# p2004dr/visual-slam

Hardware: AMD Instinct MI355X
Metric: frames/sec (extract+match+pose) at 640×480, 2000 ORB, 1/2/4/8 MI355X (higher is better)
Workload: dtype u8

## Files before the change

### visual-slam_amd/csrc/ctx.hip

```cpp
#include <algorithm>
#include <cmath>
#include <cstring>
#include <vector>

#include <cstdlib>

#include "common.h"

int mo_fail(mo_ctx* c, int code, const std::string& msg) {
    if (c) c->err = msg;
    return code;
}

static std::string g_create_err;

extern "C" int mo_abi_version(void) { return MO_ABI_VERSION; }

extern "C" int mo_device_count(void) {
    int n = 0;
    if (hipGetDeviceCount(&n) != hipSuccess) return 0;
    return n;
}

extern "C" mo_ctx* mo_create(int device, int max_w, int max_h, int max_batch) {
// ... 104 lines not shown
        float v = 0;
        hipEventElapsedTime(&v, t.ev[i], t.ev[i + 1]);
        ms[i] = v;
    }
    t.names[t.n_stages] = nullptr;
    if (names) *names = t.names;
    return n;
}

extern "C" int mo_stage_times(mo_ctx* c, const char*** names, float* ms, int cap) { return mo_stage_times_back(c, 0, names, ms, cap); }

static bool params_equal(const mo_orb_params& a, const mo_orb_params& b) {
    return std::memcmp(&a, &b, sizeof(a)) == 0;
}

static int fill_plan(mo_ctx* c, const mo_orb_params* p, int w, int h, int batch);

int mo_build_plan(mo_ctx* c, const mo_orb_params* p, int w, int h, int batch) {
    if (!p) return mo_fail(c, MO_ERR_ARG, "params is NULL");
    if (w < 64 || h < 64 || w > c->max_w || h > c->max_h)
        return mo_fail(c, MO_ERR_ARG, "image size outside the context's max_w/max_h (or < 64)");
    if (batch < 1 || batch > c->max_batch) return mo_fail(c, MO_ERR_ARG, "batch outside 1..max_batch");
    if (p->nlevels < 1 || p->nlevels > MO_MAX_LEVELS) return mo_fail(c, MO_ERR_ARG, "nlevels must be 1..12");
    if (p->first_level != 0 || p->wta_k != 2 || p->score_type != 0 || p->patch_size != 31)
        return mo_fail(c, MO_ERR_UNSUPPORTED,
                       "only firstLevel=0, WTA_K=2, HARRIS_SCORE, patchSize=31 (the reference's values) are built");
    if (p->edge_threshold < 19 || p->edge_threshold > 1024)
        return mo_fail(c, MO_ERR_UNSUPPORTED, "edge_threshold must be >= 19 (descriptor radius)");
    if (p->nfeatures < 1 || !(p->scale_factor > 1.0f) || p->scale_factor > 2.0f)
        return mo_fail(c, MO_ERR_ARG, "nfeatures >= 1, 1 < scale_factor <= 2");
    if (p->select_order != MO_ORDER_LIBSTDCXX && p->select_order != MO_ORDER_MSVC)
        return mo_fail(c, MO_ERR_ARG, "select_order must be MO_ORDER_LIBSTDCXX or MO_ORDER_MSVC");

    const bool same_key = c->plan_valid && params_equal(c->plan_params, *p) && c->plan.w == w && c->plan.h == h;
    const bool same = same_key && !c->fin_slack_dirty;
    if (!same_key)
        for (int L = 0; L < MO_MAX_LEVELS; L++) c->fin_slack[L] = 1;
    if (same && batch <= c->pb.batch_alloc) return MO_OK;
    HIPCHK(c, hipStreamSynchronize(c->stream));
    free_plan_buffers(c);
    const int rc = fill_plan(c, p, w, h, batch);
    if (rc) free_plan_buffers(c);
    return rc;
}

static int fill_plan(mo_ctx* c, const mo_orb_params* p, int w, int h, int batch) {
    Plan& P = c->plan;
    PlanBufs& pb = c->pb;
    const char* why = "";
    if (int rc = plan_geometry(P, pb, p, w, h, c->max_batch, c->fin_slack, &why)) return mo_fail(c, rc, why);

    std::vector<uint32_t> blk;
    plan_build_tables(P, pb, blk);
    int rc;
    if ((rc = pb.d_tables.upload(c, blk))) return rc;
    const int nl = P.nlevels;
    pb.rb_margin = mo_blur_margin(P.edge_threshold);
    pb.rb_pyr_margin = mo_pyr_margin(P.edge_threshold);
    pb.rb_ok = nl >= 2;
    for (int L = 1; L < nl && pb.rb_ok; L++) {
        const PlanTables::Resize& t = pb.rs[L];
        pb.rb_ok = t.two_pass_ok && orb_plan_resize_blur(P, L, &blk[t.xpk], t.ypk - t.xpk, &blk[t.ypk], t.xofs - t.ypk, pb.rb_pyr_margin, pb.rb_margin);
    }

    size_t B = (size_t)batch;
    if ((rc = pb.d_pyr.reserve_exact(c, B * P.pyr_stride)) || (rc = pb.d_blur.reserve_exact(c, B * P.blur_stride)) ||
        (rc = pb.d_cand.reserve_exact(c, B * P.cand_stride)) || (rc = pb.d_strip_cnt.reserve_exact(c, B * P.strips_per_frame)) ||
        (rc = pb.d_scratch.reserve_exact(c, B * pb.scratch_stride)))
        return rc;
    if (pb.d_fin.reserve_exact(c, B * P.fin_stride) != MO_OK)
        return mo_fail(c, MO_ERR_HIP, "hipMalloc of the final-keypoint slots failed: " + std::to_string(B * P.fin_stride * sizeof(FinalKp)) +
                                          " bytes (" + std::to_string(batch) + " frames x " + std::to_string(P.fin_stride) + " slots; slots grow with response ties)");
    if ((rc = pb.d_fin_cnt.reserve_exact(c, B * MO_MAX_LEVELS))) return rc;
    if ((rc = pb.d_dtodo.reserve_exact(c, 1 + (size_t)pb.n_dtiles * B * DT_SPLIT_LATENCY))) return rc;
    HIPCHK(c, hipMemsetAsync(pb.d_dtodo, 0, sizeof(int), c->stream));
    if ((rc = fs_build(c))) return rc;
    pb.batch_alloc = batch;
    c->plan_params = *p;
    c->plan_valid = true;
    c->fin_slack_dirty = false;
    return MO_OK;
}
```

### visual-slam_amd/csrc/orb_kernels.hip

```cpp
#include <cstring>

#include "common.h"
#include "select_replay.h"
#include "fast_score.h"

__constant__ __attribute__((aligned(16))) int8_t c_pattern[256 * 4] = {
#include "orb_pattern.inc"
};

#define WAVE 64

__device__ __forceinline__ int reflect101(int p, int len) {
    if (len == 1) return 0;
    while (p < 0 || p >= len) p = p < 0 ? -p : 2 * len - 2 - p;
    return p;
}

__device__ __forceinline__ void xcd_map(uint32_t lin, uint32_t per, uint32_t inv_per, uint32_t batch, int& frame, int& item) {
    const uint32_t b8 = batch & ~7u, cut = per * b8;
    const bool head = lin < cut;
    const uint32_t n = head ? lin >> 3 : lin - cut;
    const uint32_t q = inv_per ? __umulhi(n, inv_per) : n;
    item = (int)(n - q * per);
    frame = (int)(head ? (lin & 7u) + 8u * q : b8 + q);
// ... 555 lines not shown
    x &= x >> 4;
    x &= m32 >> 8;
    return (x & 0xFFFFu) != 0;
}

__device__ __forceinline__ int arc_score(const int d[16]) {
    int m2[16], m4[16], best = -1000;
#pragma unroll
    for (int i = 0; i < 16; i++) m2[i] = min(d[i], d[(i + 1) & 15]);
#pragma unroll
    for (int i = 0; i < 16; i++) m4[i] = min(m2[i], m2[(i + 2) & 15]);
#pragma unroll
    for (int i = 0; i < 16; i++) {
        int m8 = min(m4[i], m4[(i + 4) & 15]);
        int m9 = min(m8, d[(i + 8) & 15]);
        best = max(best, m9);
    }
    return best - 1;
}

#define FAST_LOAD_D(d, v, p, TW)                                                                              \
    d[0] = v - p[3 * TW];   d[1] = v - p[3 * TW + 1];   d[2] = v - p[2 * TW + 2];   d[3] = v - p[TW + 3];        \
    d[4] = v - p[3];        d[5] = v - p[-TW + 3];      d[6] = v - p[-2 * TW + 2];  d[7] = v - p[-3 * TW + 1];   \
    d[8] = v - p[-3 * TW];  d[9] = v - p[-3 * TW - 1];  d[10] = v - p[-2 * TW - 2]; d[11] = v - p[-TW - 3];      \
    d[12] = v - p[-3];      d[13] = v - p[TW - 3];      d[14] = v - p[2 * TW - 2];  d[15] = v - p[3 * TW - 1];

typedef short s16x2 __attribute__((ext_vector_type(2)));
__device__ __forceinline__ s16x2 pk_min(s16x2 a, s16x2 b) { return __builtin_elementwise_min(a, b); }
__device__ __forceinline__ s16x2 pk_max(s16x2 a, s16x2 b) { return __builtin_elementwise_max(a, b); }

__device__ __forceinline__ int sub16(int a, int b) { int r; asm("v_sub_u16 %0, %1, %2" : "=v"(r) : "v"(a), "v"(b)); return r; }
__device__ __forceinline__ int min16(int a, int b) { int r; asm("v_min_i16 %0, %1, %2" : "=v"(r) : "v"(a), "v"(b)); return r; }
__device__ __forceinline__ int max16(int a, int b) { int r; asm("v_max_i16 %0, %1, %2" : "=v"(r) : "v"(a), "v"(b)); return r; }
__device__ __forceinline__ int add16(int a, int b) { int r; asm("v_add_u16 %0, %1, %2" : "=v"(r) : "v"(a), "v"(b)); return r; }
__device__ __forceinline__ int min16u(int a, int b) { int r; asm("v_min_u16 %0, %1, %2" : "=v"(r) : "v"(a), "v"(b)); return r; }
__device__ __forceinline__ int max16u(int a, int b) { int r; asm("v_max_u16 %0, %1, %2" : "=v"(r) : "v"(a), "v"(b)); return r; }
__device__ __forceinline__ unsigned long long ballot_gt16(int a, int b) {
    unsigned long long m;
    asm("v_cmp_gt_i16 %0, %1, %2" : "=s"(m) : "v"(a), "v"(b));
    return m;
}

__device__ __forceinline__ void lds_store_u16_masked(unsigned long long mask, uint32_t addr, uint32_t val) {
    unsigned long long keep;
    asm volatile("s_mov_b64 %0, exec\n\ts_and_b64 exec, exec, %1\n\tds_write_b16 %2, %3\n\ts_mov_b64 exec, %0"
                 : "=&s"(keep) : "s"(mask), "v"(addr), "v"(val) : "memory", "scc");
}

#define FAST_KEEP_WORDS 512
#define FAST_STACK 384
#define FAST_NMS_Q 128

template <int TW, int NT>
__global__ __launch_bounds__(NT) void k_fast(Plan P, const uint32_t* __restrict__ strip_tab, uint32_t inv_per, int strip0,
                                              const uint8_t* __restrict__ gray, const uint8_t* __restrict__ pyr,
                                              uint32_t* __restrict__ cand, int* __restrict__ strip_cnt, int score_bytes) {
    extern __shared__ __attribute__((aligned(16))) uint8_t smem[];
    int strip = blockIdx.x, frame = blockIdx.y;
    xcd_map(blockIdx.x + gridDim.x * blockIdx.y, gridDim.x, inv_per, gridDim.y, frame, strip);
    const uint32_t se = strip_tab[strip0 + strip];
    const int L = se & 0xFF;
    const LevelInfo lv = P.lv[L];
    strip = (int)(se >> 8);
    if (strip >= lv.nstrips) return;
    const int R = lv.strip_rows;
    const int y0 = lv.by0 + strip * R;
    const int rows = min(R, lv.by0 + lv.bh - y0);
    const int SW = lv.bw + 2;
    const int xs0 = lv.bx0 - 1;
    uint8_t* s_score = smem;
    uint8_t* s_tile = smem + score_bytes;
    constexpr int NW = NT / 64;
    __shared__ int s_wsum[NW];
    __shared__ __attribute__((aligned(16))) uint16_t s_wq[NW][FAST_STACK];
    uint32_t* const s_keep = (uint32_t*)&s_wq[0][0];
    static_assert(sizeof(uint16_t) * NW * FAST_STACK >= 4 * FAST_KEEP_WORDS + sizeof(uint16_t) * NW * FAST_NMS_Q, "bitmap and queues overlay the stacks");
    const uint8_t* img = level_ptr(P, L, gray, pyr, frame);
    const int t = P.fast_threshold;
    const int tid = threadIdx.x, lane = tid & 63;
    const int wv = __builtin_amdgcn_readfirstlane(tid >> 6);

    const bool al16 = (lv.pitch & 15) == 0 && (((size_t)img) & 15) == 0;
    const bool al4 = (lv.pitch & 3) == 0 && (((size_t)img) & 3) == 0;
    const int gx0 = al16 ? (xs0 - 3) & ~15 : (xs0 - 3) & ~3, lead = xs0 - 3 - gx0;
    const int th = rows + 8, gy0 = y0 - 4;
    if (al16) {
        const int tw16 = (SW + 6 + lead + 15) >> 4;
        const uint32_t inv = 0xFFFFFFFFu / (uint32_t)tw16 + 1u;
        for (int i = tid; i < th * tw16; i += NT) {
            const int r = tw16 > 1 ? (int)__umulhi((uint32_t)i, inv) : i, c16 = i - r * tw16;
            *(uint4*)(s_tile + r * TW + 16 * c16) = *(const uint4*)(img + (size_t)(gy0 + r) * lv.pitch + gx0 + 16 * c16);
        }
    } else if (al4) {
        const int tw4 = (SW + 6 + lead + 3) >> 2;
        for (int r = wv; r < th; r += NW) {
            const uint32_t* src = (const uint32_t*)(img + (size_t)(gy0 + r) * lv.pitch + gx0);
            uint32_t* dst = (uint32_t*)(s_tile + r * TW);
            for (int c4 = lane; c4 < tw4; c4 += 64) dst[c4] = src[c4];
        }
    } else {
        const int tw_used = (SW + 6 + lead + 3) & ~3;
        for (int r = wv; r < th; r += NW) {
            const uint8_t* src = img + (size_t)(gy0 + r) * lv.pitch + gx0;
            for (int cc = lane; cc < tw_used; cc += 64) s_tile[r * TW + cc] = (gx0 + cc < lv.w) ? src[cc] : 0;
        }
    }
    for (int i = tid; i < ((rows + 2) * SW + 3) >> 2; i += NT) ((uint32_t*)s_score)[i] = 0;
    __syncthreads();

    typedef const volatile __attribute__((address_space(3))) uint8_t lds_cvu8;
    const int xbits = R > 8 ? 11 : 12;
    const uint32_t xmask = (1u << xbits) - 1u;
    auto score_one = [&](uint32_t e, int flip, bool own) {
        const int r = e >> xbits, x = e & xmask;
        const int pos = r * SW + x;
        lds_cvu8* p = (lds_cvu8*)&s_tile[(r + 3) * TW + x + 3 + lead];
        const int v = (int)p[0];
        int q[16];
#define FAST_P(k, o) q[k] = (int)p[o];
        FAST_P(0, 3 * TW)        FAST_P(1, 3 * TW + 1)    FAST_P(2, 2 * TW + 2)    FAST_P(3, TW + 3)
        FAST_P(4, 3)             FAST_P(5, -TW + 3)       FAST_P(6, -2 * TW + 2)   FAST_P(7, -3 * TW + 1)
        FAST_P(8, -3 * TW)       FAST_P(9, -3 * TW - 1)   FAST_P(10, -2 * TW - 2)  FAST_P(11, -TW - 3)
        FAST_P(12, -3)           FAST_P(13, TW - 3)       FAST_P(14, 2 * TW - 2)   FAST_P(15, 3 * TW - 1)
#undef FAST_P
        auto mn = [](int a, int b2) { return min16u(a, b2); };
        auto mx = [](int a, int b2) { return max16u(a, b2); };
        const int L = flip ? sub16(fast_arc_extreme(q, mn, mx), v) : sub16(v, fast_arc_extreme(q, mx, mn));
        const int b = (int)(short)L;
        if (own && b > t) s_score[pos] = (uint8_t)(b - 1);
    };
    {
        uint16_t* wq = s_wq[wv];
        const int nxc = (SW + 63) >> 6;
        int qd = 0, qb = 0;
        int ra = 0, ja = wv, rb = 0, jb = wv + NW;
        while (ja >= nxc) { ja -= nxc; ra++; }
        while (jb >= nxc) { jb -= nxc; rb++; }
        const int tv = t;
        auto chunk = [&](int r, int j) {
            const int x = (j << 6) + lane;
            const int rem = SW - (j << 6);
            const unsigned long long valid = rem >= 64 ? ~0ull : (1ull << rem) - 1ull;
            const uint8_t* w = &s_tile[r * TW + lead + min(x, SW - 1)];
            const int v = w[3 * TW + 3];
            const int p0 = w[6 * TW + 3], p4 = w[3 * TW + 6], p8 = w[3], p12 = w[3 * TW];
            const int pair_hi = min16u(min16u(max16u(p0, p4), max16u(p4, p8)), min16u(max16u(p8, p12), max16u(p12, p0)));
            const int pair_lo = max16u(max16u(min16u(p0, p4), min16u(p4, p8)), max16u(min16u(p8, p12), min16u(p12, p0)));
            const unsigned long long md = ballot_gt16(sub16(v, tv), pair_hi) & valid;
            const unsigned long long mb = ballot_gt16(pair_lo, add16(v, tv)) & valid;
            const uint32_t e = (uint32_t)((r << xbits) | x);
            const uint32_t wq_lds = (uint32_t)(uintptr_t)wq;
            lds_store_u16_masked(md, wq_lds + 2u * (uint32_t)(qd + __builtin_amdgcn_mbcnt_hi((unsigned)(md >> 32), __builtin_amdgcn_mbcnt_lo((unsigned)md, 0u))), e);
            qd += __popcll(md);
            lds_store_u16_masked(mb, wq_lds + 2u * (uint32_t)(FAST_STACK - 1 - qb - (int)__builtin_amdgcn_mbcnt_hi((unsigned)(mb >> 32), __builtin_amdgcn_mbcnt_lo((unsigned)mb, 0u))), e);
            qb += __popcll(mb);
        };
        while (ra < rows + 2) {
            chunk(ra, ja);
            if (rb < rows + 2) chunk(rb, jb);
            if (qd >= 64 || qb >= 64) {
                replay::wave_sync();
                while (qd >= 64) { qd -= 64; score_one(wq[qd + lane], 0, true); }
                while (qb >= 64) { qb -= 64; score_one(wq[FAST_STACK - 1 - qb - lane], 0xFF, true); }
                replay::wave_sync();
            }
            ja += 2 * NW;
            while (ja >= nxc) { ja -= nxc; ra++; }
            jb += 2 * NW;
            while (jb >= nxc) { jb -= nxc; rb++; }
        }
        replay::wave_sync();
        if (qd > 0) score_one(wq[min(lane, qd - 1)], 0, lane < qd);
        if (qb > 0) score_one(wq[FAST_STACK - 1 - min(lane, qb - 1)], 0xFF, lane < qb);
    }
    __syncthreads();
    for (int i = tid; i < FAST_KEEP_WORDS; i += NT) s_keep[i] = 0;
    __syncthreads();

    const int nitems = rows * lv.bw;
    {
        const uint32_t inv_sw = 0xFFFFFFFFu / (uint32_t)SW + 1u;
        auto nms_at = [&](int p) {
            const int r = (int)__umulhi((uint32_t)p, inv_sw), x = p - r * SW;
            if (r < 1 || r > rows || x < 1 || x > lv.bw) return;
            const uint8_t* c = &s_score[p];
            const int mid = c[0];
            const int nb = max16u(max16u(max16u((int)c[-SW - 1], (int)c[-SW]), max16u((int)c[-SW + 1], (int)c[-1])),
                                  max16u(max16u((int)c[1], (int)c[SW - 1]), max16u((int)c[SW], (int)c[SW + 1])));
            if ((uint16_t)mid > (uint16_t)nb) {
                const int i = (r - 1) * lv.bw + (x - 1);
                atomicOr(&s_keep[i >> 5], 1u << (i & 31));
            }
        };
        uint16_t* const nq = (uint16_t*)(s_keep + FAST_KEEP_WORDS) + wv * FAST_NMS_Q;
        const uint32_t nq_lds = (uint32_t)(uintptr_t)nq;
        const int k_end = ((rows + 1) * SW + 3) >> 2;
        int qn = 0;
        for (int k0 = (SW >> 2) + (wv << 6); k0 < k_end; k0 += NT) {
            const int k = k0 + lane;
            const uint32_t w = k < k_end ? ((const uint32_t*)s_score)[k] : 0u;
#pragma unroll
            for (int bq = 0; bq < 4; bq++) {
                const unsigned long long m = __ballot((w & (0xFFu << (8 * bq))) != 0u);
                lds_store_u16_masked(m, nq_lds + 2u * (uint32_t)(qn + __builtin_amdgcn_mbcnt_hi((unsigned)(m >> 32), __builtin_amdgcn_mbcnt_lo((unsigned)m, 0u))),
                                     (uint32_t)(4 * k + bq));
                qn += __popcll(m);
                if (qn >= 64) {
                    replay::wave_sync();
                    qn -= 64;
                    nms_at(nq[qn + lane]);
                    replay::wave_sync();
                }
            }
        }
        replay::wave_sync();
        if (lane < qn) nms_at(nq[lane]);
    }
    __syncthreads();
    const int nwords = (nitems + 31) >> 5, wpt = (nwords + NT - 1) / NT;
    uint32_t kw[2] = {0u, 0u};
#pragma unroll
    for (int q = 0; q < 2; q++)
        if (q < wpt && tid * wpt + q < nwords) kw[q] = s_keep[tid * wpt + q];
    const int cnt = __popc(kw[0]) + __popc(kw[1]);
    int incl = cnt;
#pragma unroll
    for (int o = 1; o < 64; o <<= 1) {
        int n = __shfl_up(incl, o, 64);
        if (lane >= o) incl += n;
    }
    if (lane == 63) s_wsum[wv] = incl;
    __syncthreads();
    int base = 0;
    for (int k = 0; k < wv; k++) base += s_wsum[k];
    int total = 0;
    for (int k = 0; k < NW; k++) total += s_wsum[k];
    int pos = base + incl - cnt;
    uint32_t* out = cand + (size_t)frame * P.cand_stride + lv.cand_off + (size_t)strip * lv.strip_cap;
#pragma unroll
    for (int q = 0; q < 2; q++) {
        uint32_t bits = kw[q];
        while (bits) {
            const int j = __ffs((int)bits) - 1;
            bits &= bits - 1;
            const int i = (tid * wpt + q) * 32 + j;
            const int rr = lv.bw > 1 ? (int)__umulhi((uint32_t)i, lv.inv_bw) : i, xx = i - rr * lv.bw;
            const int sc = s_score[(rr + 1) * SW + xx + 1];
            if (pos < lv.strip_cap) out[pos] = ((uint32_t)sc << 24) | ((uint32_t)(y0 + rr) << 12) | (uint32_t)(lv.bx0 + xx);
            pos++;
        }
    }
    if (tid == 0) strip_cnt[(size_t)frame * P.strips_per_frame + lv.strip_base + strip] = min(total, lv.strip_cap);
}

template <int TW, int NT> static int launch_fast_tw(mo_ctx* c, const uint8_t* d_gray, int batch, int strip0, int nstrips) {
    const Plan& P = c->plan;
    const size_t score_bytes = c->pb.score_bytes, lds = score_bytes + (size_t)(c->pb.max_rows + 8) * TW + 16;
    if (int rc = mo_raise_dyn_lds(c, (const void*)k_fast<TW, NT>, 128 * 1024)) return rc;
    const uint32_t per = (uint32_t)nstrips, inv_per = per > 1 ? 0xFFFFFFFFu / per + 1u : 0u;
    hipLaunchKernelGGL((k_fast<TW, NT>), dim3(nstrips, batch), dim3(NT), lds, c->stream, P, c->pb.d_tables + c->pb.strip_tab, inv_per, strip0, d_gray,
                       c->pb.d_pyr, c->pb.d_cand, c->pb.d_strip_cnt, (int)score_bytes);
    HIPCHK(c, hipGetLastError());
    return MO_OK;
}

int orb_launch_fast(mo_ctx* c, const uint8_t* d_gray, int batch, int level_lo, int level_hi) {
    const Plan& P = c->plan;
    level_lo = std::max(level_lo, 0); level_hi = std::min(level_hi, P.nlevels);
    if (level_lo >= level_hi) return MO_OK;
    const int strip0 = P.lv[level_lo].strip_base;
    const int nstrips = (level_hi < P.nlevels ? P.lv[level_hi].strip_base : P.strips_per_frame) - strip0;
    if (nstrips < 1) return MO_OK;
    switch (mo_fast_tw(c->pb.tw_need)) {
    case 608: return launch_fast_tw<608, 256>(c, d_gray, batch, strip0, nstrips);
    case 704: return launch_fast_tw<704, 256>(c, d_gray, batch, strip0, nstrips);
    case 1344: return launch_fast_tw<1344, 256>(c, d_gray, batch, strip0, nstrips);
    case 2112: return launch_fast_tw<2112, 256>(c, d_gray, batch, strip0, nstrips);
    default: return launch_fast_tw<4160, 256>(c, d_gray, batch, strip0, nstrips);
    }
}

#ifndef SEL_BUF_KB
#define SEL_BUF_KB 46
#endif
#define SEL_BUF_BYTES (SEL_BUF_KB * 1024)

__device__ float harris_response(const uint8_t* img, int pitch, int x0, int y0) {
    int a = 0, b = 0, cc = 0;
    for (int i = -3; i <= 3; i++) {
        const uint8_t* pm = img + (size_t)(y0 + i - 1) * pitch + x0;
        const uint8_t* p0 = pm + pitch;
        const uint8_t* pp = p0 + pitch;
#pragma unroll
        for (int j = -3; j <= 3; j++) {
            int Ix = ((int)p0[j + 1] - (int)p0[j - 1]) * 2 + ((int)pm[j + 1] - (int)pm[j - 1]) +
                     ((int)pp[j + 1] - (int)pp[j - 1]);
            int Iy = ((int)pp[j] - (int)pm[j]) * 2 + ((int)pp[j - 1] - (int)pm[j - 1]) + ((int)pp[j + 1] - (int)pm[j + 1]);
            a += Ix * Ix;
            b += Iy * Iy;
            cc += Ix * Iy;
        }
    }
    const float scale = 1.f / ((1 << 2) * 7 * 255.f);
    const float scale_sq_sq = scale * scale * scale * scale;
    float fa = (float)a, fb = (float)b, fc = (float)cc;
    float t1 = fa * fb;
    float t2 = fc * fc;
    float s = fa + fb;
    float t3 = 0.04f * s;
    float t4 = t3 * s;
    return ((t1 - t2) - t4) * scale_sq_sq;
}

__device__ __forceinline__ size_t sel_need_bytes(int n, int rec_bytes) {
    return (((size_t)n * rec_bytes + 7) & ~(size_t)7) + ((((size_t)n / 2 + 1) * 2 + 7) & ~(size_t)7) + ((size_t)n / 64 + 8) * 8;
}

#define HG 8
#define SEL_THREADS 256
#define SEL_THREADS_LATENCY 1024

__device__ __forceinline__ void harris_fetch(const uint8_t* img, int pitch, int x0, int y0, int g, uint32_t (&reg)[4]) {
    const uint8_t* base = img + (size_t)(y0 - 4) * pitch + ((x0 - 4) & ~3);
#pragma unroll
    for (int k = 0; k < 4; k++) {
        const int q = min(g + HG * k, 26), r = q / 3, dw = q - 3 * r;
        reg[k] = *(const uint32_t*)(base + r * pitch + 4 * dw);
    }
}
__device__ __forceinline__ float harris_group(const uint32_t (&reg)[4], int x0, uint32_t* tile , int g) {
    const int off = (x0 - 4) & 3;
// ... 691 lines not shown
```

### visual-slam_amd/csrc/plan_tables.h

```cpp
#pragma once
#include <algorithm>
#include <cmath>
#include <cstring>
#include <stdint.h>
#include <vector>

#include "../../include/vslam_amd.h"

#define MO_MAX_LEVELS 12
#define MO_HALF_PATCH 15
#define MO_STRIP_ROWS 8
#ifndef MO_STRIP_ROWS_LATENCY
#define MO_STRIP_ROWS_LATENCY 2
#endif
#define SEL_MAXSTRIPS 2047

#define BT_W 64
#define BT_H 58
#ifndef DT_W
#define DT_W 128
#endif
#define DT_H 64
#ifndef DT_SPLIT_LATENCY
#define DT_SPLIT_LATENCY 4
#endif

struct LevelInfo {
    int w, h, pitch;
    int off;
    int bpitch, boff;
    float scale;
    int quota;
    int bx0, by0, bw, bh;
    uint32_t inv_bw;
    int strip_rows;
    int nstrips;
    int strip_cap;
    int strip_base;
    int cand_off;
    int cand_cap;
    int fin_off, fin_cap;
    int scr_off;
};

struct Plan {
    int w, h, nlevels;
    int edge_threshold, fast_threshold, select_order, nfeatures;
    int pyr_stride;
    int blur_stride;
    int strips_per_frame;
    int cand_stride;
    int fin_stride;
    int umax[MO_HALF_PATCH + 1];
    int gk[7];
    LevelInfo lv[MO_MAX_LEVELS];
};

inline int mo_blur_margin(int edge_threshold) { return (edge_threshold - 19) & ~3; }
inline int mo_pyr_margin(int edge_threshold) { return std::max(mo_blur_margin(edge_threshold) - 4, 0); }

static inline size_t mo_align(size_t v, size_t a) { return (v + a - 1) & ~(a - 1); }

static inline int mo_fast_tw(int tw_need) { return tw_need <= 608 ? 608 : tw_need <= 704 ? 704 : tw_need <= 1344 ? 1344 : tw_need <= 2112 ? 2112 : 4160; }

struct PlanTables {
    size_t scratch_stride = 0;
    size_t score_bytes = 0;
    int tw_need = 0, max_rows = 1;
    int max_strips = 1;
    struct Resize {
        uint32_t xpk = 0, ypk = 0, xofs = 0, xc1 = 0, yofs = 0, yc1 = 0;
        bool two_pass_ok = true;
    } rs[MO_MAX_LEVELS];
    uint32_t tile_tab[2] = {};
    int tile_cum[2][MO_MAX_LEVELS + 1] = {};
    uint32_t strip_tab = 0;
    uint32_t dtile_tab = 0, dtile_icw = 0;
    int n_dtiles = 0;
};

static inline int cv_round_f(float v) { return (int)lrintf(v); }
static inline int cv_round_d(double v) { return (int)lrint(v); }
static inline int align_up(int v, int a) { return (v + a - 1) / a * a; }

inline void mo_linear_coeffs(int srcsize, int dstsize, std::vector<int>& ofs, std::vector<int>& c1) {
    ofs.assign(dstsize, 0);
    c1.assign(dstsize, 0);
    double inv_scale = (double)dstsize / (double)srcsize;
    double scale = 1.0 / inv_scale;
    int minofst = 0, maxofst = dstsize;
    for (int val = 0; val < dstsize; val++) {
        double fval = scale * ((double)val + 0.5) - 0.5;
        int ival = (int)std::floor(fval);
        if (ival >= 0 && srcsize > 1) {
            if (ival < srcsize - 1) {
                ofs[val] = ival;
                c1[val] = cv_round_d((fval - (double)ival) * 256.0);
            } else {
                ofs[val] = srcsize - 1;
                maxofst = std::min(maxofst, val);
            }
        } else {
            minofst = std::max(minofst, val + 1);
        }
    }
    for (int val = 0; val < dstsize; val++) {
        if (val < minofst) { ofs[val] = 0; c1[val] = 0; }
        if (val >= maxofst) { ofs[val] = srcsize - 1; c1[val] = 0; }
    }
}

inline int plan_geometry(Plan& P, PlanTables& T, const mo_orb_params* p, int w, int h, int max_batch, const int* fin_slack, const char** why) {
    std::memset(&P, 0, sizeof(P));
    P.w = w; P.h = h; P.nlevels = p->nlevels;
    P.edge_threshold = p->edge_threshold;
    P.fast_threshold = std::min(std::max(p->fast_threshold, 0), 255);
    P.select_order = p->select_order;
    P.nfeatures = p->nfeatures;

    int nl = p->nlevels;
    {
        float factor = (float)(1.0 / (double)p->scale_factor);
        float nd = p->nfeatures * (1 - factor) / (1 - (float)std::pow((double)factor, (double)nl));
        int sum = 0;
        for (int L = 0; L < nl - 1; L++) {
            P.lv[L].quota = cv_round_f(nd);
            sum += P.lv[L].quota;
            nd *= factor;
        }
// ... 28 lines not shown
        LevelInfo& v = P.lv[L];
        v.scale = (float)std::pow((double)p->scale_factor, (double)L);
        float inv_scale = 1.0f / v.scale;
        v.w = cv_round_f((float)w * inv_scale);
        v.h = cv_round_f((float)h * inv_scale);
        if (v.w < 1 || v.h < 1) { *why = "pyramid level collapses to zero size; reduce nlevels"; return MO_ERR_ARG; }
        if (L == 0) { v.pitch = w; v.off = 0; }
        else {
            v.pitch = align_up(v.w, 16);
            v.off = pyr_off;
            pyr_off += align_up(v.pitch * v.h, 256);
        }
        v.bpitch = align_up(v.w, 16);
        v.boff = blur_off;
        blur_off += align_up(v.bpitch * v.h, 256);
        if (v.w <= 2 * et || v.h <= 2 * et) { v.bx0 = v.by0 = et; v.bw = v.bh = 0; }
        else { v.bx0 = et; v.by0 = et; v.bw = v.w - 2 * et; v.bh = v.h - 2 * et; }
        v.inv_bw = v.bw > 1 ? 0xFFFFFFFFu / (uint32_t)v.bw + 1u : 0u;
        v.strip_rows = max_batch <= 2 ? MO_STRIP_ROWS_LATENCY : MO_STRIP_ROWS;
        while (v.strip_rows > 1 && v.strip_rows * v.bw > 16384) v.strip_rows /= 2;
        while (v.strip_rows < MO_STRIP_ROWS && v.bh > 0 && (v.bh + v.strip_rows - 1) / v.strip_rows > SEL_MAXSTRIPS && 2 * v.strip_rows * v.bw <= 16384)
            v.strip_rows *= 2;
        if (v.bw > 16384) { *why = "level too wide"; return MO_ERR_UNSUPPORTED; }
        v.nstrips = v.bh > 0 ? (v.bh + v.strip_rows - 1) / v.strip_rows : 0;
        v.strip_cap = ((v.strip_rows + 1) / 2) * ((v.bw + 1) / 2);
        v.strip_base = strip_base;
        strip_base += v.nstrips;
        v.cand_off = cand_off;
        v.cand_cap = v.nstrips * v.strip_cap;
        cand_off += v.cand_cap;
        v.fin_off = fin_off;
        v.fin_cap = (int)std::max<long long>(1, std::min<long long>(v.cand_cap, (4ll * v.quota + 256) * fin_slack[L]));
        fin_off += v.fin_cap;
        v.scr_off = scr_off;
        scr_off += v.cand_cap + (v.cand_cap + 1) / 2 + (v.cand_cap / 2 + 8) / 4 + 2 + v.cand_cap / 64 + 12;
    }
    P.pyr_stride = std::max(pyr_off, 256);
    P.blur_stride = blur_off;
    P.strips_per_frame = std::max(strip_base, 1);
    P.cand_stride = std::max(cand_off, 1);
    P.fin_stride = fin_off;
    T.scratch_stride = (size_t)scr_off;

    T.score_bytes = 0; T.tw_need = 0; T.max_rows = 1; T.max_strips = 1;
    for (int L = 0; L < nl; L++) {
        const LevelInfo& v = P.lv[L];
        T.score_bytes = std::max(T.score_bytes, (((size_t)(v.strip_rows + 2) * (v.bw + 2) + 15) & ~(size_t)15));
        T.tw_need = std::max(T.tw_need, (v.bw + 2 + 6 + 15 + 15) & ~15);
        T.max_rows = std::max(T.max_rows, v.strip_rows);
        T.max_strips = std::max(T.max_strips, v.nstrips);
    }
    if (T.score_bytes + (size_t)(T.max_rows + 8) * mo_fast_tw(T.tw_need) + 16 > 128 * 1024) { *why = "level too wide for the FAST strip kernel"; return MO_ERR_UNSUPPORTED; }
    if (T.max_strips > SEL_MAXSTRIPS) { *why = "too many strips per level"; return MO_ERR_UNSUPPORTED; }
    return MO_OK;
}

inline void plan_build_tables(const Plan& P, PlanTables& T, std::vector<uint32_t>& blk) {
    auto start = [&blk]() { blk.resize(mo_align(blk.size(), 64), 0u); return (uint32_t)blk.size(); };
    blk.clear();
    for (int L = 1; L < P.nlevels; L++) {
        std::vector<int> xo, xc, yo, yc;
        mo_linear_coeffs(P.lv[L - 1].w, P.lv[L].w, xo, xc);
        mo_linear_coeffs(P.lv[L - 1].h, P.lv[L].h, yo, yc);
        const int dw = P.lv[L].w, dh = P.lv[L].h, wp = ((dw + 63) & ~63) + 64, hp = ((dh + 63) & ~63) + 64;
        auto pack = [](const std::vector<int>& o, const std::vector<int>& c1, int srcsize, int padded) {
            std::vector<uint32_t> t((size_t)padded);
            for (int i = 0; i < padded; i++) {
                const int j = std::min(i, (int)o.size() - 1), o1 = std::min(o[j] + 1, srcsize - 1);
                t[i] = (uint32_t)o[j] | ((uint32_t)(o1 - o[j]) << 15) | ((uint32_t)c1[j] << 16);
            }
            return t;
        };
        const std::vector<uint32_t> xp = pack(xo, xc, P.lv[L - 1].w, wp), yp = pack(yo, yc, P.lv[L - 1].h, hp);
        bool window_ok = true;
        for (int x = 0; x < dw && window_ok; x++) {
            const int xl = std::min(x + 3, dw - 1);
            window_ok = std::min(xo[xl] + 1, P.lv[L - 1].w - 1) - xo[x] <= 7;
        }
        PlanTables::Resize& t = T.rs[L];
        t.two_pass_ok = window_ok;
        t.xpk = start(); t.ypk = t.xpk + wp;
        t.xofs = t.ypk + hp; t.xc1 = t.xofs + dw; t.yofs = t.xc1 + dw; t.yc1 = t.yofs + dh;
        blk.insert(blk.end(), xp.begin(), xp.end());
        blk.insert(blk.end(), yp.begin(), yp.end());
        for (const std::vector<int>* v : {&xo, &xc, &yo, &yc}) blk.insert(blk.end(), v->begin(), v->end());
    }
    for (int slot = 0; slot < 2; slot++) {
        const int margin = slot ? mo_blur_margin(P.edge_threshold) : 0;
        const uint32_t t0 = T.tile_tab[slot] = start();
        for (int L = 0; L < P.nlevels; L++) {
            const int cw = std::max(P.lv[L].w - 2 * margin, 1), chh = std::max(P.lv[L].h - 2 * margin, 1);
            const int tx = (cw + BT_W - 1) / BT_W, ty = (chh + BT_H - 1) / BT_H;
            T.tile_cum[slot][L] = (int)(blk.size() - t0);
            for (int y = 0; y < ty; y++)
                for (int x = 0; x < tx; x++) blk.push_back((uint32_t)L | ((uint32_t)x << 8) | ((uint32_t)y << 20));
        }
        T.tile_cum[slot][P.nlevels] = (int)(blk.size() - t0);
    }
    T.strip_tab = start();
    blk.resize(blk.size() + (size_t)P.strips_per_frame, 0xFFFFFF00u);
    for (int L = 0; L < P.nlevels; L++)
        for (int st = 0; st < P.lv[L].nstrips; st++) blk[T.strip_tab + (size_t)P.lv[L].strip_base + st] = (uint32_t)L | ((uint32_t)st << 8);
    T.dtile_tab = start();
    for (int L = 0; L < P.nlevels; L++)
        for (int y = 0; y < (P.lv[L].bh + DT_H - 1) / DT_H; y++)
            for (int x = 0; x < (P.lv[L].bw + DT_W - 1) / DT_W; x++) blk.push_back((uint32_t)L | ((uint32_t)x << 8) | ((uint32_t)y << 20));
    T.n_dtiles = (int)(blk.size() - T.dtile_tab);
// ... 16 lines not shown
```

Measured before the change: 118,900.

## Chain consecutive FAST strips per block to reuse halo rows in LDS

Lets one FAST block process a run of consecutive strips of a level. Between strips it copies the 8-row halo of the image tile and the two-row border of the score buffer within LDS instead of reloading them from global memory. A new chain table built at plan time replaces the strip table, and the kernel gains a waves-per-EU occupancy attribute. The default chain length is 1, so the reuse path stays inactive unless the macro is raised. The occupancy attribute may also cap register use.

```diff
diff --git a/visual-slam_amd/csrc/ctx.hip b/visual-slam_amd/csrc/ctx.hip
--- a/visual-slam_amd/csrc/ctx.hip
+++ b/visual-slam_amd/csrc/ctx.hip
@@ -180,6 +180,7 @@
 
     std::vector<uint32_t> blk;
     plan_build_tables(P, pb, blk);
+    plan_build_chain_table(P, pb, blk);
     int rc;
     if ((rc = pb.d_tables.upload(c, blk))) return rc;
     const int nl = P.nlevels;
diff --git a/visual-slam_amd/csrc/orb_kernels.hip b/visual-slam_amd/csrc/orb_kernels.hip
--- a/visual-slam_amd/csrc/orb_kernels.hip
+++ b/visual-slam_amd/csrc/orb_kernels.hip
@@ -631,20 +631,18 @@
 #define FAST_NMS_Q 128
 
 template <int TW, int NT>
-__global__ __launch_bounds__(NT) void k_fast(Plan P, const uint32_t* __restrict__ strip_tab, uint32_t inv_per, int strip0,
+__global__ __launch_bounds__(NT) __attribute__((amdgpu_waves_per_eu(8, 8))) void k_fast(Plan P, const uint32_t* __restrict__ chain_tab, uint32_t inv_per, int chain0,
                                               const uint8_t* __restrict__ gray, const uint8_t* __restrict__ pyr,
                                               uint32_t* __restrict__ cand, int* __restrict__ strip_cnt, int score_bytes) {
     extern __shared__ __attribute__((aligned(16))) uint8_t smem[];
-    int strip = blockIdx.x, frame = blockIdx.y;
-    xcd_map(blockIdx.x + gridDim.x * blockIdx.y, gridDim.x, inv_per, gridDim.y, frame, strip);
-    const uint32_t se = strip_tab[strip0 + strip];
-    const int L = se & 0xFF;
+    int chain = blockIdx.x, frame = blockIdx.y;
+    xcd_map(blockIdx.x + gridDim.x * blockIdx.y, gridDim.x, inv_per, gridDim.y, frame, chain);
+    const uint32_t ce = chain_tab[chain0 + chain];
+    const int L = ce & 0xFF;
     const LevelInfo lv = P.lv[L];
-    strip = (int)(se >> 8);
-    if (strip >= lv.nstrips) return;
+    const int strip_first = (int)((ce >> 8) & 0xFFFu), nchain = (int)(ce >> 20);
+    if (nchain < 1) return;
     const int R = lv.strip_rows;
-    const int y0 = lv.by0 + strip * R;
-    const int rows = min(R, lv.by0 + lv.bh - y0);
     const int SW = lv.bw + 2;
     const int xs0 = lv.bx0 - 1;
     uint8_t* s_score = smem;
@@ -662,182 +660,211 @@
     const bool al16 = (lv.pitch & 15) == 0 && (((size_t)img) & 15) == 0;
     const bool al4 = (lv.pitch & 3) == 0 && (((size_t)img) & 3) == 0;
     const int gx0 = al16 ? (xs0 - 3) & ~15 : (xs0 - 3) & ~3, lead = xs0 - 3 - gx0;
-    const int th = rows + 8, gy0 = y0 - 4;
-    if (al16) {
-        const int tw16 = (SW + 6 + lead + 15) >> 4;
-        const uint32_t inv = 0xFFFFFFFFu / (uint32_t)tw16 + 1u;
-        for (int i = tid; i < th * tw16; i += NT) {
-            const int r = tw16 > 1 ? (int)__umulhi((uint32_t)i, inv) : i, c16 = i - r * tw16;
-            *(uint4*)(s_tile + r * TW + 16 * c16) = *(const uint4*)(img + (size_t)(gy0 + r) * lv.pitch + gx0 + 16 * c16);
-        }
-    } else if (al4) {
-        const int tw4 = (SW + 6 + lead + 3) >> 2;
-        for (int r = wv; r < th; r += NW) {
-            const uint32_t* src = (const uint32_t*)(img + (size_t)(gy0 + r) * lv.pitch + gx0);
-            uint32_t* dst = (uint32_t*)(s_tile + r * TW);
-            for (int c4 = lane; c4 < tw4; c4 += 64) dst[c4] = src[c4];
-        }
-    } else {
-        const int tw_used = (SW + 6 + lead + 3) & ~3;
-        for (int r = wv; r < th; r += NW) {
-            const uint8_t* src = img + (size_t)(gy0 + r) * lv.pitch + gx0;
-            for (int cc = lane; cc < tw_used; cc += 64) s_tile[r * TW + cc] = (gx0 + cc < lv.w) ? src[cc] : 0;
-        }
-    }
-    for (int i = tid; i < ((rows + 2) * SW + 3) >> 2; i += NT) ((uint32_t*)s_score)[i] = 0;
-    __syncthreads();
-
-    typedef const volatile __attribute__((address_space(3))) uint8_t lds_cvu8;
-    const int xbits = R > 8 ? 11 : 12;
-    const uint32_t xmask = (1u << xbits) - 1u;
-    auto score_one = [&](uint32_t e, int flip, bool own) {
-        const int r = e >> xbits, x = e & xmask;
-        const int pos = r * SW + x;
-        lds_cvu8* p = (lds_cvu8*)&s_tile[(r + 3) * TW + x + 3 + lead];
-        const int v = (int)p[0];
-        int q[16];
-#define FAST_P(k, o) q[k] = (int)p[o];
-        FAST_P(0, 3 * TW)        FAST_P(1, 3 * TW + 1)    FAST_P(2, 2 * TW + 2)    FAST_P(3, TW + 3)
-        FAST_P(4, 3)             FAST_P(5, -TW + 3)       FAST_P(6, -2 * TW + 2)   FAST_P(7, -3 * TW + 1)
-        FAST_P(8, -3 * TW)       FAST_P(9, -3 * TW - 1)   FAST_P(10, -2 * TW - 2)  FAST_P(11, -TW - 3)
-        FAST_P(12, -3)           FAST_P(13, TW - 3)       FAST_P(14, 2 * TW - 2)   FAST_P(15, 3 * TW - 1)
-#undef FAST_P
-        auto mn = [](int a, int b2) { return min16u(a, b2); };
-        auto mx = [](int a, int b2) { return max16u(a, b2); };
-        const int L = flip ? sub16(fast_arc_extreme(q, mn, mx), v) : sub16(v, fast_arc_extreme(q, mx, mn));
-        const int b = (int)(short)L;
-        if (own && b > t) s_score[pos] = (uint8_t)(b - 1);
+    const int tw16 = (SW + 6 + lead + 15) >> 4;
+    const uint32_t inv16 = 0xFFFFFFFFu / (uint32_t)tw16 + 1u;
+    auto stage = [&](int r_lo, int r_hi, int gy0) {
+        if (al16) {
+            for (int i = tid; i < (r_hi - r_lo) * tw16; i += NT) {
+                const int q = tw16 > 1 ? (int)__umulhi((uint32_t)i, inv16) : i, c16 = i - q * tw16, r = r_lo + q;
+                *(uint4*)(s_tile + r * TW + 16 * c16) = *(const uint4*)(img + (size_t)(gy0 + r) * lv.pitch + gx0 + 16 * c16);
+            }
+        } else if (al4) {
+            const int tw4 = (SW + 6 + lead + 3) >> 2;
+            for (int r = r_lo + wv; r < r_hi; r += NW) {
+                const uint32_t* src = (const uint32_t*)(img + (size_t)(gy0 + r) * lv.pitch + gx0);
+                uint32_t* dst = (uint32_t*)(s_tile + r * TW);
+                for (int c4 = lane; c4 < tw4; c4 += 64) dst[c4] = src[c4];
+            }
+        } else {
+            const int tw_used = (SW + 6 + lead + 3) & ~3;
+            for (int r = r_lo + wv; r < r_hi; r += NW) {
+                const uint8_t* src = img + (size_t)(gy0 + r) * lv.pitch + gx0;
+                for (int cc = lane; cc < tw_used; cc += 64) s_tile[r * TW + cc] = (gx0 + cc < lv.w) ? src[cc] : 0;
+            }
+        }
     };
-    {
-        uint16_t* wq = s_wq[wv];
-        const int nxc = (SW + 63) >> 6;
-        int qd = 0, qb = 0;
-        int ra = 0, ja = wv, rb = 0, jb = wv + NW;
-        while (ja >= nxc) { ja -= nxc; ra++; }
-        while (jb >= nxc) { jb -= nxc; rb++; }
-        const int tv = t;
-        auto chunk = [&](int r, int j) {
-            const int x = (j << 6) + lane;
-            const int rem = SW - (j << 6);
-            const unsigned long long valid = rem >= 64 ? ~0ull : (1ull << rem) - 1ull;
-            const uint8_t* w = &s_tile[r * TW + lead + min(x, SW - 1)];
-            const int v = w[3 * TW + 3];
-            const int p0 = w[6 * TW + 3], p4 = w[3 * TW + 6], p8 = w[3], p12 = w[3 * TW];
-            const int pair_hi = min16u(min16u(max16u(p0, p4), max16u(p4, p8)), min16u(max16u(p8, p12), max16u(p12, p0)));
-            const int pair_lo = max16u(max16u(min16u(p0, p4), min16u(p4, p8)), max16u(min16u(p8, p12), min16u(p12, p0)));
-            const unsigned long long md = ballot_gt16(sub16(v, tv), pair_hi) & valid;
-            const unsigned long long mb = ballot_gt16(pair_lo, add16(v, tv)) & valid;
-            const uint32_t e = (uint32_t)((r << xbits) | x);
-            const uint32_t wq_lds = (uint32_t)(uintptr_t)wq;
-            lds_store_u16_masked(md, wq_lds + 2u * (uint32_t)(qd + __builtin_amdgcn_mbcnt_hi((unsigned)(md >> 32), __builtin_amdgcn_mbcnt_lo((unsigned)md, 0u))), e);
-            qd += __popcll(md);
-            lds_store_u16_masked(mb, wq_lds + 2u * (uint32_t)(FAST_STACK - 1 - qb - (int)__builtin_amdgcn_mbcnt_hi((unsigned)(mb >> 32), __builtin_amdgcn_mbcnt_lo((unsigned)mb, 0u))), e);
-            qb += __popcll(mb);
+
+    for (int s = 0;; s++) {
+        const int strip = strip_first + s;
+        const int y0 = lv.by0 + strip * R;
+        const int rows = min(R, lv.by0 + lv.bh - y0);
+        const int rows_nx = s + 1 < nchain ? min(R, lv.by0 + lv.bh - (y0 + rows)) : 0;
+        if (s == 0) {
+            stage(0, rows + 8, y0 - 4);
+            for (int i = tid; i < ((rows + 2) * SW + 3) >> 2; i += NT) ((uint32_t*)s_score)[i] = 0;
+        } else {
+            uint32_t* const sc = (uint32_t*)s_score;
+            const int src4 = (R * SW) >> 2, n2 = (2 * SW + 3) >> 2;
+            const uint32_t last_mask = ((2 * SW) & 2) ? 0xFFFFu : 0xFFFFFFFFu;
+            for (int i = tid; i < n2; i += NT) {
+                const uint32_t v = sc[src4 + i];
+                sc[src4 + i] = 0u;
+                sc[i] = i == n2 - 1 ? v & last_mask : v;
+            }
+            for (int i = n2 + tid; i < ((rows + 2) * SW + 3) >> 2; i += NT)
+                if (i < src4 || i >= src4 + n2) sc[i] = 0u;
+        }
+        __syncthreads();
+
+        typedef const volatile __attribute__((address_space(3))) uint8_t lds_cvu8;
+        const int xbits = R > 8 ? 11 : 12;
+        const uint32_t xmask = (1u << xbits) - 1u;
+        auto score_one = [&](uint32_t e, int flip, bool own) {
+            const int r = e >> xbits, x = e & xmask;
+            const int pos = r * SW + x;
+            lds_cvu8* p = (lds_cvu8*)&s_tile[(r + 3) * TW + x + 3 + lead];
+            const int v = (int)p[0];
+            int q[16];
+    #define FAST_P(k, o) q[k] = (int)p[o];
+            FAST_P(0, 3 * TW)        FAST_P(1, 3 * TW + 1)    FAST_P(2, 2 * TW + 2)    FAST_P(3, TW + 3)
+            FAST_P(4, 3)             FAST_P(5, -TW + 3)       FAST_P(6, -2 * TW + 2)   FAST_P(7, -3 * TW + 1)
+            FAST_P(8, -3 * TW)       FAST_P(9, -3 * TW - 1)   FAST_P(10, -2 * TW - 2)  FAST_P(11, -TW - 3)
+            FAST_P(12, -3)           FAST_P(13, TW - 3)       FAST_P(14, 2 * TW - 2)   FAST_P(15, 3 * TW - 1)
+    #undef FAST_P
+            auto mn = [](int a, int b2) { return min16u(a, b2); };
+            auto mx = [](int a, int b2) { return max16u(a, b2); };
+            const int L = flip ? sub16(fast_arc_extreme(q, mn, mx), v) : sub16(v, fast_arc_extreme(q, mx, mn));
+            const int b = (int)(short)L;
+            if (own && b > t) s_score[pos] = (uint8_t)(b - 1);
         };
-        while (ra < rows + 2) {
-            chunk(ra, ja);
-            if (rb < rows + 2) chunk(rb, jb);
-            if (qd >= 64 || qb >= 64) {
-                replay::wave_sync();
-                while (qd >= 64) { qd -= 64; score_one(wq[qd + lane], 0, true); }
-                while (qb >= 64) { qb -= 64; score_one(wq[FAST_STACK - 1 - qb - lane], 0xFF, true); }
-                replay::wave_sync();
-            }
-            ja += 2 * NW;
+        {
+            uint16_t* wq = s_wq[wv];
+            const int nxc = (SW + 63) >> 6;
+            int qd = 0, qb = 0;
+            const int r_first = s ? 2 : 0;
+            int ra = r_first, ja = wv, rb = r_first, jb = wv + NW;
             while (ja >= nxc) { ja -= nxc; ra++; }
-            jb += 2 * NW;
             while (jb >= nxc) { jb -= nxc; rb++; }
-        }
-        replay::wave_sync();
-        if (qd > 0) score_one(wq[min(lane, qd - 1)], 0, lane < qd);
-        if (qb > 0) score_one(wq[FAST_STACK - 1 - min(lane, qb - 1)], 0xFF, lane < qb);
-    }
-    __syncthreads();
-    for (int i = tid; i < FAST_KEEP_WORDS; i += NT) s_keep[i] = 0;
-    __syncthreads();
-
-    const int nitems = rows * lv.bw;
-    {
-        const uint32_t inv_sw = 0xFFFFFFFFu / (uint32_t)SW + 1u;
-        auto nms_at = [&](int p) {
-            const int r = (int)__umulhi((uint32_t)p, inv_sw), x = p - r * SW;
-            if (r < 1 || r > rows || x < 1 || x > lv.bw) return;
-            const uint8_t* c = &s_score[p];
-            const int mid = c[0];
-            const int nb = max16u(max16u(max16u((int)c[-SW - 1], (int)c[-SW]), max16u((int)c[-SW + 1], (int)c[-1])),
-                                  max16u(max16u((int)c[1], (int)c[SW - 1]), max16u((int)c[SW], (int)c[SW + 1])));
-            if ((uint16_t)mid > (uint16_t)nb) {
-                const int i = (r - 1) * lv.bw + (x - 1);
-                atomicOr(&s_keep[i >> 5], 1u << (i & 31));
-            }
-        };
-        uint16_t* const nq = (uint16_t*)(s_keep + FAST_KEEP_WORDS) + wv * FAST_NMS_Q;
-        const uint32_t nq_lds = (uint32_t)(uintptr_t)nq;
-        const int k_end = ((rows + 1) * SW + 3) >> 2;
-        int qn = 0;
-        for (int k0 = (SW >> 2) + (wv << 6); k0 < k_end; k0 += NT) {
-            const int k = k0 + lane;
-            const uint32_t w = k < k_end ? ((const uint32_t*)s_score)[k] : 0u;
-#pragma unroll
-            for (int bq = 0; bq < 4; bq++) {
-                const unsigned long long m = __ballot((w & (0xFFu << (8 * bq))) != 0u);
-                lds_store_u16_masked(m, nq_lds + 2u * (uint32_t)(qn + __builtin_amdgcn_mbcnt_hi((unsigned)(m >> 32), __builtin_amdgcn_mbcnt_lo((unsigned)m, 0u))),
-                                     (uint32_t)(4 * k + bq));
-                qn += __popcll(m);
-                if (qn >= 64) {
+            const int tv = t;
+            auto chunk = [&](int r, int j) {
+                const int x = (j << 6) + lane;
+                const int rem = SW - (j << 6);
+                const unsigned long long valid = rem >= 64 ? ~0ull : (1ull << rem) - 1ull;
+                const uint8_t* w = &s_tile[r * TW + lead + min(x, SW - 1)];
+                const int v = w[3 * TW + 3];
+                const int p0 = w[6 * TW + 3], p4 = w[3 * TW + 6], p8 = w[3], p12 = w[3 * TW];
+                const int pair_hi = min16u(min16u(max16u(p0, p4), max16u(p4, p8)), min16u(max16u(p8, p12), max16u(p12, p0)));
+                const int pair_lo = max16u(max16u(min16u(p0, p4), min16u(p4, p8)), max16u(min16u(p8, p12), min16u(p12, p0)));
+                const unsigned long long md = ballot_gt16(sub16(v, tv), pair_hi) & valid;
+                const unsigned long long mb = ballot_gt16(pair_lo, add16(v, tv)) & valid;
+                const uint32_t e = (uint32_t)((r << xbits) | x);
+                const uint32_t wq_lds = (uint32_t)(uintptr_t)wq;
+                lds_store_u16_masked(md, wq_lds + 2u * (uint32_t)(qd + __builtin_amdgcn_mbcnt_hi((unsigned)(md >> 32), __builtin_amdgcn_mbcnt_lo((unsigned)md, 0u))), e);
+                qd += __popcll(md);
+                lds_store_u16_masked(mb, wq_lds + 2u * (uint32_t)(FAST_STACK - 1 - qb - (int)__builtin_amdgcn_mbcnt_hi((unsigned)(mb >> 32), __builtin_amdgcn_mbcnt_lo((unsigned)mb, 0u))), e);
+                qb += __popcll(mb);
+            };
+            while (ra < rows + 2) {
+                chunk(ra, ja);
+                if (rb < rows + 2) chunk(rb, jb);
+                if (qd >= 64 || qb >= 64) {
                     replay::wave_sync();
-                    qn -= 64;
-                    nms_at(nq[qn + lane]);
+                    while (qd >= 64) { qd -= 64; score_one(wq[qd + lane], 0, true); }
+                    while (qb >= 64) { qb -= 64; score_one(wq[FAST_STACK - 1 - qb - lane], 0xFF, true); }
                     replay::wave_sync();
                 }
-            }
-        }
-        replay::wave_sync();
-        if (lane < qn) nms_at(nq[lane]);
-    }
-    __syncthreads();
-    const int nwords = (nitems + 31) >> 5, wpt = (nwords + NT - 1) / NT;
-    uint32_t kw[2] = {0u, 0u};
-#pragma unroll
-    for (int q = 0; q < 2; q++)
-        if (q < wpt && tid * wpt + q < nwords) kw[q] = s_keep[tid * wpt + q];
-    const int cnt = __popc(kw[0]) + __popc(kw[1]);
-    int incl = cnt;
-#pragma unroll
-    for (int o = 1; o < 64; o <<= 1) {
-        int n = __shfl_up(incl, o, 64);
-        if (lane >= o) incl += n;
-    }
-    if (lane == 63) s_wsum[wv] = incl;
-    __syncthreads();
-    int base = 0;
-    for (int k = 0; k < wv; k++) base += s_wsum[k];
-    int total = 0;
-    for (int k = 0; k < NW; k++) total += s_wsum[k];
-    int pos = base + incl - cnt;
-    uint32_t* out = cand + (size_t)frame * P.cand_stride + lv.cand_off + (size_t)strip * lv.strip_cap;
-#pragma unroll
-    for (int q = 0; q < 2; q++) {
-        uint32_t bits = kw[q];
-        while (bits) {
-            const int j = __ffs((int)bits) - 1;
-            bits &= bits - 1;
-            const int i = (tid * wpt + q) * 32 + j;
-            const int rr = lv.bw > 1 ? (int)__umulhi((uint32_t)i, lv.inv_bw) : i, xx = i - rr * lv.bw;
-            const int sc = s_score[(rr + 1) * SW + xx + 1];
-            if (pos < lv.strip_cap) out[pos] = ((uint32_t)sc << 24) | ((uint32_t)(y0 + rr) << 12) | (uint32_t)(lv.bx0 + xx);
-            pos++;
-        }
-    }
-    if (tid == 0) strip_cnt[(size_t)frame * P.strips_per_frame + lv.strip_base + strip] = min(total, lv.strip_cap);
-}
-
-template <int TW, int NT> static int launch_fast_tw(mo_ctx* c, const uint8_t* d_gray, int batch, int strip0, int nstrips) {
+                ja += 2 * NW;
+                while (ja >= nxc) { ja -= nxc; ra++; }
+                jb += 2 * NW;
+                while (jb >= nxc) { jb -= nxc; rb++; }
+            }
+            replay::wave_sync();
+            if (qd > 0) score_one(wq[min(lane, qd - 1)], 0, lane < qd);
+            if (qb > 0) score_one(wq[FAST_STACK - 1 - min(lane, qb - 1)], 0xFF, lane < qb);
+        }
+        __syncthreads();
+        for (int i = tid; i < FAST_KEEP_WORDS; i += NT) s_keep[i] = 0;
+        if (rows_nx > 0)
+            for (int r = wv; r < 8; r += NW)
+                for (int c16 = lane; c16 < tw16; c16 += 64) *(uint4*)(s_tile + r * TW + 16 * c16) = *(const uint4*)(s_tile + (r + rows) * TW + 16 * c16);
+        __syncthreads();
+        if (rows_nx > 0) stage(8, 8 + rows_nx, y0 + rows - 4);
+
+        const int nitems = rows * lv.bw;
+        {
+            const uint32_t inv_sw = 0xFFFFFFFFu / (uint32_t)SW + 1u;
+            auto nms_at = [&](int p) {
+                const int r = (int)__umulhi((uint32_t)p, inv_sw), x = p - r * SW;
+                if (r < 1 || r > rows || x < 1 || x > lv.bw) return;
+                const uint8_t* c = &s_score[p];
+                const int mid = c[0];
+                const int nb = max16u(max16u(max16u((int)c[-SW - 1], (int)c[-SW]), max16u((int)c[-SW + 1], (int)c[-1])),
+                                      max16u(max16u((int)c[1], (int)c[SW - 1]), max16u((int)c[SW], (int)c[SW + 1])));
+                if ((uint16_t)mid > (uint16_t)nb) {
+                    const int i = (r - 1) * lv.bw + (x - 1);
+                    atomicOr(&s_keep[i >> 5], 1u << (i & 31));
+                }
+            };
+            uint16_t* const nq = (uint16_t*)(s_keep + FAST_KEEP_WORDS) + wv * FAST_NMS_Q;
+            const uint32_t nq_lds = (uint32_t)(uintptr_t)nq;
+            const int k_end = ((rows + 1) * SW + 3) >> 2;
+            int qn = 0;
+            for (int k0 = (SW >> 2) + (wv << 6); k0 < k_end; k0 += NT) {
+                const int k = k0 + lane;
+                const uint32_t w = k < k_end ? ((const uint32_t*)s_score)[k] : 0u;
+    #pragma unroll
+                for (int bq = 0; bq < 4; bq++) {
+                    const unsigned long long m = __ballot((w & (0xFFu << (8 * bq))) != 0u);
+                    lds_store_u16_masked(m, nq_lds + 2u * (uint32_t)(qn + __builtin_amdgcn_mbcnt_hi((unsigned)(m >> 32), __builtin_amdgcn_mbcnt_lo((unsigned)m, 0u))),
+                                         (uint32_t)(4 * k + bq));
+                    qn += __popcll(m);
+                    if (qn >= 64) {
+                        replay::wave_sync();
+                        qn -= 64;
+                        nms_at(nq[qn + lane]);
+                        replay::wave_sync();
+                    }
+                }
+            }
+            replay::wave_sync();
+            if (lane < qn) nms_at(nq[lane]);
+        }
+        __syncthreads();
+        const int nwords = (nitems + 31) >> 5, wpt = (nwords + NT - 1) / NT;
+        uint32_t kw[2] = {0u, 0u};
+    #pragma unroll
+        for (int q = 0; q < 2; q++)
+            if (q < wpt && tid * wpt + q < nwords) kw[q] = s_keep[tid * wpt + q];
+        const int cnt = __popc(kw[0]) + __popc(kw[1]);
+        int incl = cnt;
+    #pragma unroll
+        for (int o = 1; o < 64; o <<= 1) {
+            int n = __shfl_up(incl, o, 64);
+            if (lane >= o) incl += n;
+        }
+        if (lane == 63) s_wsum[wv] = incl;
+        __syncthreads();
+        int base = 0;
+        for (int k = 0; k < wv; k++) base += s_wsum[k];
+        int total = 0;
+        for (int k = 0; k < NW; k++) total += s_wsum[k];
+        int pos = base + incl - cnt;
+        uint32_t* out = cand + (size_t)frame * P.cand_stride + lv.cand_off + (size_t)strip * lv.strip_cap;
+    #pragma unroll
+        for (int q = 0; q < 2; q++) {
+            uint32_t bits = kw[q];
+            while (bits) {
+                const int j = __ffs((int)bits) - 1;
+                bits &= bits - 1;
+                const int i = (tid * wpt + q) * 32 + j;
+                const int rr = lv.bw > 1 ? (int)__umulhi((uint32_t)i, lv.inv_bw) : i, xx = i - rr * lv.bw;
+                const int sc = s_score[(rr + 1) * SW + xx + 1];
+                if (pos < lv.strip_cap) out[pos] = ((uint32_t)sc << 24) | ((uint32_t)(y0 + rr) << 12) | (uint32_t)(lv.bx0 + xx);
+                pos++;
+            }
+        }
+        if (tid == 0) strip_cnt[(size_t)frame * P.strips_per_frame + lv.strip_base + strip] = min(total, lv.strip_cap);
+        if (rows_nx == 0) break;
+        __syncthreads();
+    }
+}
+
+template <int TW, int NT> static int launch_fast_tw(mo_ctx* c, const uint8_t* d_gray, int batch, int chain0, int nchains) {
     const Plan& P = c->plan;
     const size_t score_bytes = c->pb.score_bytes, lds = score_bytes + (size_t)(c->pb.max_rows + 8) * TW + 16;
     if (int rc = mo_raise_dyn_lds(c, (const void*)k_fast<TW, NT>, 128 * 1024)) return rc;
-    const uint32_t per = (uint32_t)nstrips, inv_per = per > 1 ? 0xFFFFFFFFu / per + 1u : 0u;
-    hipLaunchKernelGGL((k_fast<TW, NT>), dim3(nstrips, batch), dim3(NT), lds, c->stream, P, c->pb.d_tables + c->pb.strip_tab, inv_per, strip0, d_gray,
+    const uint32_t per = (uint32_t)nchains, inv_per = per > 1 ? 0xFFFFFFFFu / per + 1u : 0u;
+    hipLaunchKernelGGL((k_fast<TW, NT>), dim3(nchains, batch), dim3(NT), lds, c->stream, P, c->pb.d_tables + c->pb.chain_tab, inv_per, chain0, d_gray,
                        c->pb.d_pyr, c->pb.d_cand, c->pb.d_strip_cnt, (int)score_bytes);
     HIPCHK(c, hipGetLastError());
     return MO_OK;
@@ -847,15 +874,14 @@
     const Plan& P = c->plan;
     level_lo = std::max(level_lo, 0); level_hi = std::min(level_hi, P.nlevels);
     if (level_lo >= level_hi) return MO_OK;
-    const int strip0 = P.lv[level_lo].strip_base;
-    const int nstrips = (level_hi < P.nlevels ? P.lv[level_hi].strip_base : P.strips_per_frame) - strip0;
-    if (nstrips < 1) return MO_OK;
+    const int chain0 = c->pb.chain_cum[level_lo], nchains = c->pb.chain_cum[level_hi] - chain0;
+    if (nchains < 1) return MO_OK;
     switch (mo_fast_tw(c->pb.tw_need)) {
-    case 608: return launch_fast_tw<608, 256>(c, d_gray, batch, strip0, nstrips);
-    case 704: return launch_fast_tw<704, 256>(c, d_gray, batch, strip0, nstrips);
-    case 1344: return launch_fast_tw<1344, 256>(c, d_gray, batch, strip0, nstrips);
-    case 2112: return launch_fast_tw<2112, 256>(c, d_gray, batch, strip0, nstrips);
-    default: return launch_fast_tw<4160, 256>(c, d_gray, batch, strip0, nstrips);
+    case 608: return launch_fast_tw<608, 256>(c, d_gray, batch, chain0, nchains);
+    case 704: return launch_fast_tw<704, 256>(c, d_gray, batch, chain0, nchains);
+    case 1344: return launch_fast_tw<1344, 256>(c, d_gray, batch, chain0, nchains);
+    case 2112: return launch_fast_tw<2112, 256>(c, d_gray, batch, chain0, nchains);
+    default: return launch_fast_tw<4160, 256>(c, d_gray, batch, chain0, nchains);
     }
 }
 
diff --git a/visual-slam_amd/csrc/plan_tables.h b/visual-slam_amd/csrc/plan_tables.h
--- a/visual-slam_amd/csrc/plan_tables.h
+++ b/visual-slam_amd/csrc/plan_tables.h
@@ -12,6 +12,9 @@
 #define MO_STRIP_ROWS 8
 #ifndef MO_STRIP_ROWS_LATENCY
 #define MO_STRIP_ROWS_LATENCY 2
+#endif
+#ifndef MO_FAST_CHAIN
+#define MO_FAST_CHAIN 1
 #endif
 #define SEL_MAXSTRIPS 2047
 
@@ -75,6 +78,9 @@
     uint32_t tile_tab[2] = {};
     int tile_cum[2][MO_MAX_LEVELS + 1] = {};
     uint32_t strip_tab = 0;
+    uint32_t chain_tab = 0;
+    int chain_len[MO_MAX_LEVELS] = {};
+    int chain_cum[MO_MAX_LEVELS + 1] = {};
     uint32_t dtile_tab = 0, dtile_icw = 0;
     int n_dtiles = 0;
 };
@@ -209,7 +215,25 @@
     }
     if (T.score_bytes + (size_t)(T.max_rows + 8) * mo_fast_tw(T.tw_need) + 16 > 128 * 1024) { *why = "level too wide for the FAST strip kernel"; return MO_ERR_UNSUPPORTED; }
     if (T.max_strips > SEL_MAXSTRIPS) { *why = "too many strips per level"; return MO_ERR_UNSUPPORTED; }
+    for (int L = 0; L < MO_MAX_LEVELS; L++) {
+        const LevelInfo& v = P.lv[L];
+        const int want = max_batch <= 2 || v.strip_rows < 8 ? 1 : MO_FAST_CHAIN > 0 ? MO_FAST_CHAIN : v.nstrips;
+        T.chain_len[L] = std::max(1, std::min(want, v.nstrips));
+    }
     return MO_OK;
+}
+
+inline void plan_build_chain_table(const Plan& P, PlanTables& T, std::vector<uint32_t>& blk) {
+    blk.resize(mo_align(blk.size(), 64), 0u);
+    T.chain_tab = (uint32_t)blk.size();
+    for (int L = 0; L < P.nlevels; L++) {
+        T.chain_cum[L] = (int)(blk.size() - T.chain_tab);
+        const int C = std::max(T.chain_len[L], 1);
+        for (int st = 0; st < P.lv[L].nstrips; st += C)
+            blk.push_back((uint32_t)L | ((uint32_t)st << 8) | ((uint32_t)std::min(C, P.lv[L].nstrips - st) << 20));
+    }
+    for (int L = P.nlevels; L <= MO_MAX_LEVELS; L++) T.chain_cum[L] = (int)(blk.size() - T.chain_tab);
+    if (blk.size() == T.chain_tab) blk.push_back(0u);
 }
 
 inline void plan_build_tables(const Plan& P, PlanTables& T, std::vector<uint32_t>& blk) {
```

New measurement: 116,900. 0.983x the previous value.
